# urw7rs/diffusion-models-made-easy

Measured on AMD Instinct MI355X. Metric: denoising steps/sec + training images/sec, DDPM UNet CIFAR10 32×32 @1/2/4/8 GPU, higher is better.
Workload: dtype bf16; 1 GPU; DDPM T=1000 sampling, CIFAR10 32x32, default UNet (32,416,643 params, random init), batch 128 per GPU, t.shape=(1,); global_batch=128, parallelism=dp1 (independent chains per GPU, no data-path collective)

## Files before the change

### diffusion-models-made-easy_amd/csrc/conv1x1_as.hip

```cpp
#include <stdio.h>

#include "conv_common.h"

namespace dmme {

typedef unsigned u32x4_as __attribute__((ext_vector_type(4)));
typedef __attribute__((address_space(3))) u32x4_as lds_u32x4_as;
typedef __attribute__((address_space(3))) f32x4 lds_f32x4_as;

__host__ __device__ constexpr int as_stage_bytes(bool res) { return res ? 128 * 256 : 128 * 128; }
__host__ __device__ constexpr int as_ring(bool res) { return res ? 2 : 3; }

__host__ __device__ inline int as_fold_bytes(int Cout) { return (Cout * 4 + 1023) & ~1023; }

__device__ __forceinline__ void as_swap32(float& x, float& y) {
#if defined(__HIP_DEVICE_COMPILE__)
    asm volatile("s_nop 1\n\tv_permlane32_swap_b32 %0, %1" : "+v"(x), "+v"(y));
#endif
}
__device__ __forceinline__ void as_mfma_drain() {
#if defined(__HIP_DEVICE_COMPILE__)
    asm volatile("s_nop 15\n\ts_nop 7" ::: "memory");
#endif
}

__device__ __forceinline__ float as_sum_rows(float s) {
    s += __builtin_bit_cast(float, __builtin_amdgcn_update_dpp(0, __builtin_bit_cast(int, s), 0x128, 0xf, 0xf, true));
    s += __builtin_bit_cast(float, __builtin_amdgcn_ds_swizzle(__builtin_bit_cast(int, s), 0x401F));
    float lo = s, hi = s;
    as_swap32(lo, hi);
    return lo + hi;
}
__device__ __forceinline__ float as_sum_slots(float s, int nv) {
    if (nv >= 2) s += __builtin_bit_cast(float, __builtin_amdgcn_update_dpp(0, __builtin_bit_cast(int, s), 0xB1, 0xf, 0xf, true));
    if (nv == 4) s += __builtin_bit_cast(float, __builtin_amdgcn_update_dpp(0, __builtin_bit_cast(int, s), 0x4E, 0xf, 0xf, true));
    return s;
}

__device__ __forceinline__ void as_barrier() {
#if defined(__HIP_DEVICE_COMPILE__)
    asm volatile("s_barrier" ::: "memory");
#endif
}

template <int K, typename T>
__device__ __forceinline__ void as_prologue_tile(char* ldsA, const float* par, int tid, bool silu, bool dm) {
    typedef typename Vec8<T>::type bf16x8;
    typedef __attribute__((address_space(3))) u32x4_as lv4;
    typedef __attribute__((address_space(3))) f32x4 lf4;
    const lds_c* P3 = (const lds_c*)par;
#pragma unroll 1
    for (int it = tid; it < 128 * (K / 8); it += 512) {
        const int piece = it & 7, row = (it >> 3) & 127, c = it >> 10;
        const int ch = c * 64 + ((piece ^ ((row >> 1) & 7)) << 3);
        lv4* p = (lv4*)(lds_c*)(ldsA + it * 16);
        bf16x8 x = __builtin_bit_cast(bf16x8, *p);
        float v[8];
#pragma unroll
        for (int e = 0; e < 8; e += 4) {
            const f32x4 sc = *(const lf4*)(P3 + (ch + e) * 4), sh = *(const lf4*)(P3 + (K + ch + e) * 4);
#pragma unroll
            for (int j = 0; j < 4; ++j) v[e + j] = fmaf((float)x[e + j], sc[j], sh[j]);
        }
        if (silu) {
#pragma unroll
            for (int e = 0; e < 8; ++e) v[e] = silu_fast(v[e]);
        }
        if (dm) {
#pragma unroll
            for (int e = 0; e < 8; e += 4) {
                const f32x4 m = *(const lf4*)(P3 + (2 * K + ch + e) * 4);
#pragma unroll
                for (int j = 0; j < 4; ++j) v[e + j] *= m[j];
            }
        }
#pragma unroll
        for (int e = 0; e < 8; ++e) x[e] = (T)v[e];
        *p = __builtin_bit_cast(u32x4_as, x);
    }
}

template <int KCH, bool RES, typename T = bf16>
__global__ void __launch_bounds__(512) conv1x1_as_kernel(ConvArgs a, int HW, int NU) {
    typedef typename Vec8<T>::type bf16x8;
    constexpr int K = 64 * KCH, NKS = 4 * KCH;
    constexpr int RING = as_ring(RES), STAGE = as_stage_bytes(RES);
    constexpr int U_BYTES = 64 * KCH * ROW_DATA;
    constexpr int DPU = 2 * KCH;
    extern __shared__ __attribute__((aligned(16))) char lds[];
    const int tid = threadIdx.x, lane = tid & 63, wave = __builtin_amdgcn_readfirstlane(tid >> 6);
#define AS_STAMP(K) do { if (a.stamps && blockIdx.x < 2 && (threadIdx.x & 255) == 0) a.stamps[blockIdx.x * 32 + (threadIdx.x >> 8) * 16 + (K)] = (long long)wall_clock64(); } while (0)
    AS_STAMP(0);
    const int p0 = blockIdx.x * 128;
    float* foldL = reinterpret_cast<float*>(lds + RING * U_BYTES);
    char* stageL = lds + RING * U_BYTES + as_fold_bytes(a.Cout);
    char* ldsA = RES ? stageL : lds + U_BYTES;
    const bool has_pro = a.scale || a.dmask || a.pro_silu;
    float* parL = reinterpret_cast<float*>(RES ? lds + U_BYTES : stageL);

    if (wave >= 4) {
        const int t = tid - 256, sw = wave - 4;
        for (int c = t; c < a.Cout; c += 256) foldL[c] = (a.bias ? a.bias[c] : 0.f) + (a.tproj ? a.tproj[c] : 0.f);
        if (has_pro && t < K) {
            const int n = p0 / HW, so = n * K + t;
            float sc = 1.f, sh = 0.f;
            if (a.has_gni) {
                gn_in_scale_shift(a, n, t, K, p0 == n * HW, sc, sh);
            } else if (a.scale) {
                sc = a.scale[so];
                sh = a.shift[so];
            }
            parL[t] = sc;
            parL[K + t] = sh;
            parL[2 * K + t] = a.dmask ? a.dmask[so] : 1.f;
        }
        wait_lgkm_all();
        as_barrier();
        if (has_pro) {
            as_prologue_tile<K, T>(ldsA, parL, tid, a.pro_silu != 0, a.dmask != nullptr);
            wait_lgkm_all();
            as_barrier();
        }
        as_barrier();
        const int slot8 = lane & 7;
        const T* res = (const T*)a.res1;
        T* dst = (T*)a.dst;
        const int cgs = a.gn_cg, nv = cgs >> 3;
        int64_t goff[4];
        int soff[4];
#pragma unroll
        for (int q = 0; q < 4; ++q) {
            const int px = 32 * sw + 8 * q + (lane >> 3);
            goff[q] = (int64_t)(p0 + px) * a.Cout + slot8 * 8;
            soff[q] = RES ? px * 256 + ((slot8 ^ (px & 7)) << 5) : px * 128 + ((slot8 ^ (px & 7)) << 4);
        }
#pragma unroll 1
        for (int u = 0; u < NU; ++u) {
            uint4 rv[4];
            if constexpr (RES) {
#pragma unroll
                for (int q = 0; q < 4; ++q) rv[q] = *reinterpret_cast<const uint4*>(res + goff[q] + u * 64);
            }
            as_barrier();
            if (u < 3) AS_STAMP(4 + 3 * u);
            const char* st = stageL + (u & 1) * STAGE;
            float xs[4][8];
            float s1 = 0.f, s1b = 0.f;
#pragma unroll
            for (int q = 0; q < 4; ++q) {
                uint4 raw;
                if constexpr (RES) {
                    const f32x4 v0 = *reinterpret_cast<const f32x4*>(st + soff[q]), v1 = *reinterpret_cast<const f32x4*>(st + soff[q] + 16);
                    const bf16x8 y = __builtin_bit_cast(bf16x8, rv[q]);
                    bf16x8 o;
#pragma unroll
                    for (int e = 0; e < 4; ++e) {
                        o[e] = (T)(v0[e] + (float)y[e]);
                        o[4 + e] = (T)(v1[e] + (float)y[4 + e]);
                    }
                    raw = __builtin_bit_cast(uint4, o);
                } else {
                    raw = *reinterpret_cast<const uint4*>(st + soff[q]);
                }
                *reinterpret_cast<uint4*>(dst + goff[q] + u * 64) = raw;
                if (a.gn_part) {
                    const bf16x8 o = __builtin_bit_cast(bf16x8, raw);
#pragma unroll
                    for (int e = 0; e < 8; ++e) {
                        xs[q][e] = (float)o[e];
                        if (e < 4) s1 += xs[q][e];
                        else s1b += xs[q][e];
                    }
                }
            }
            if (a.gn_part && cgs == 4) {
                const float meanA = as_sum_rows(s1) * (1.f / 128.f), meanB = as_sum_rows(s1b) * (1.f / 128.f);
                float qa = 0.f, qb = 0.f;
#pragma unroll
                for (int q = 0; q < 4; ++q)
#pragma unroll
                    for (int e = 0; e < 4; ++e) {
                        const float da = xs[q][e] - meanA, db = xs[q][4 + e] - meanB;
                        qa = fmaf(da, da, qa);
                        qb = fmaf(db, db, qb);
                    }
                const float m2A = as_sum_rows(qa), m2B = as_sum_rows(qb);
                if (lane < 8) {
                    const int pw = p0 + 32 * sw, n = pw / HW, tile_s = (pw - n * HW) >> 5;
                    const int G = a.Cout / 4, g_first = (u * 64 + lane * 8) / 4;
                    float* o = a.gn_part + (((int64_t)n * a.gn_tiles + tile_s) * G + g_first) * 2;
                    *reinterpret_cast<f32x4*>(o) = f32x4{meanA, m2A, meanB, m2B};
                }
            } else if (a.gn_part) {
                s1 += s1b;
                const float mean = as_sum_slots(as_sum_rows(s1), nv) * (1.f / (float)(32 * cgs));
                float q2 = 0.f;
#pragma unroll
                for (int q = 0; q < 4; ++q)
#pragma unroll
                    for (int e = 0; e < 8; ++e) {
                        const float d = xs[q][e] - mean;
                        q2 = fmaf(d, d, q2);
                    }
                const float m2 = as_sum_slots(as_sum_rows(q2), nv);
                if (lane < 8 && (lane & (nv - 1)) == 0) {
                    const int pw = p0 + 32 * sw, n = pw / HW, tile_s = (pw - n * HW) >> 5;
                    const int G = a.Cout / cgs, c_first = u * 64 + lane * 8;
                    float* o = a.gn_part + (((int64_t)n * a.gn_tiles + tile_s) * G + c_first / cgs) * 2;
                    *reinterpret_cast<f32x2*>(o) = f32x2{mean, m2};
                }
            }
            if (u < 3) AS_STAMP(5 + 3 * u);
        }
        AS_STAMP(13);
        return;
    }

    const int r = lane & 31, h = lane >> 5;
    const int pm = wave >> 1, cn = wave & 1;
    const unsigned ring_base = (unsigned)__builtin_amdgcn_readfirstlane((int)(unsigned)(size_t)(lds_c*)lds);
    const unsigned a_base = (unsigned)__builtin_amdgcn_readfirstlane((int)(unsigned)(size_t)(lds_c*)ldsA);
    unsigned boff[DPU];
#pragma unroll
    for (int i = 0; i < DPU; ++i) {
        const int I = wave + 4 * i, c = I >> 3, row = 8 * (I & 7) + (lane >> 3);
        boff[i] = (unsigned)(row * K + c * 64 + ((lane & 7) ^ ((row >> 1) & 7)) * 8) * 2u;
    }
    auto dma_unit = [&](int u, int slot) __attribute__((always_inline)) {
        const char* sb = (const char*)a.w + (int64_t)u * 64 * K * 2;
#pragma unroll
        for (int i = 0; i < DPU; ++i) glds16_hidden_s(sb, boff[i], ring_base + (unsigned)(slot * U_BYTES + (wave + 4 * i) * 1024));
    };
#pragma unroll
    for (int i = 0; i < 4 * KCH; ++i) {
        const int I = wave + 4 * i, c = I >> 4, row = 8 * (I & 15) + (lane >> 3);
        const int c0 = c * 64;
        const bool second = c0 >= a.C1;
        const T* sbase = second ? (const T*)a.src2 : (const T*)a.src1;
        const int Cs = second ? a.C2 : a.C1, cb = second ? c0 - a.C1 : c0;
        glds16_hidden(sbase + (int64_t)(p0 + row) * Cs + cb + ((lane & 7) ^ ((row >> 1) & 7)) * 8, a_base + (unsigned)(I * 1024));
    }
    dma_unit(0, 0);
    AS_STAMP(1);
    wait_vm_keep<0>();
    as_barrier();
    AS_STAMP(2);

    if (has_pro) {
        as_prologue_tile<K, T>(ldsA, parL, tid, a.pro_silu != 0, a.dmask != nullptr);
        wait_lgkm_all();
        as_barrier();
    }
    uint4 af[2][NKS];
    {
        const lds_c* A3 = (const lds_c*)ldsA;
#pragma unroll
        for (int mi = 0; mi < 2; ++mi) {
            const int row = pm * 64 + mi * 32 + r;
            const int t = row * ROW_DATA + ((h ^ ((row >> 1) & 7)) << 4);
#pragma unroll
            for (int ks = 0; ks < NKS; ++ks)
                af[mi][ks] = __builtin_bit_cast(uint4, *reinterpret_cast<const lds_u32x4_as*>(A3 + (ks >> 2) * (128 * ROW_DATA) + (t ^ ((ks & 3) << 5))));
        }
    }
    AS_STAMP(3);
    wait_vm_keep<0>();
    as_barrier();
    if (NU > 1) dma_unit(1, 1);
    if (RING > 2 && NU > 2) dma_unit(2, 2);

    const int tB = (cn * 32 + r) * ROW_DATA + ((h ^ (((cn * 32 + r) >> 1) & 7)) << 4);
    uint4 bfr[2][4];
#define AS_READ(SET, SLOT, KG)                                                                                                     \
    do {                                                                                                                           \
        const lds_c* rb_ = (const lds_c*)(size_t)(ring_base + (unsigned)((SLOT) * U_BYTES + (KG) * (64 * ROW_DATA)));              \
        _Pragma("unroll") for (int kk = 0; kk < 4; ++kk)                                                                           \
            bfr[SET][kk] = __builtin_bit_cast(uint4, *reinterpret_cast<const lds_u32x4_as*>(rb_ + (tB ^ (kk << 5))));               \
    } while (0)
    const lds_c* F3 = (const lds_c*)foldL;
    f32x16 fold;
#define AS_FOLD(U)                                                                                                                 \
    _Pragma("unroll") for (int g = 0; g < 4; ++g) {                                                                                \
        const f32x4 t_ = *reinterpret_cast<const lds_f32x4_as*>(F3 + ((U) * 64 + cn * 32 + 8 * g + 4 * h) * 4);                    \
        fold[4 * g] = t_[0];                                                                                                       \
        fold[4 * g + 1] = t_[1];                                                                                                   \
        fold[4 * g + 2] = t_[2];                                                                                                   \
        fold[4 * g + 3] = t_[3];                                                                                                   \
    }
    AS_READ(0, 0, 0);
    AS_FOLD(0);
    int slot = 0;
    const int px = pm * 64 + lane;
    char* stw = stageL + px * (RES ? 256 : 128);
    int stoff[4];
#pragma unroll
    for (int g = 0; g < 4; ++g) stoff[g] = ((cn * 4 + g) ^ (px & 7)) << (RES ? 5 : 4);
#pragma unroll 1
    for (int u = 0; u < NU; ++u) {
        const int nslot = slot == RING - 1 ? 0 : slot + 1;
        f32x16 acc[2];
#pragma unroll
        for (int kg = 0; kg < KCH; ++kg) {
            if (kg + 1 < KCH) {
                if (kg & 1)
                    AS_READ(0, slot, kg + 1);
                else
                    AS_READ(1, slot, kg + 1);
            }
#pragma unroll
            for (int kk = 0; kk < 4; ++kk)
#pragma unroll
                for (int mi = 0; mi < 2; ++mi)
                {
                    if (kg == 0 && kk == 0) acc[mi] = fold;
                    mma16<T>(__builtin_bit_cast(uint4, bfr[kg & 1][kk]), __builtin_bit_cast(uint4, af[mi][4 * kg + kk]), acc[mi]);
                }
        }
        if (u < 3) AS_STAMP(4 + 3 * u);
        char* st = stw + (u & 1) * STAGE;
        as_mfma_drain();
#pragma unroll
        for (int g = 0; g < 4; ++g) {
            float v[8];
#pragma unroll
            for (int i = 0; i < 4; ++i) {
                float x = acc[0][4 * g + i], y = acc[1][4 * g + i];
                as_swap32(x, y);
                v[i] = x;
                v[4 + i] = y;
            }
            if constexpr (RES) {
                *reinterpret_cast<f32x4*>(st + stoff[g]) = f32x4{v[0], v[1], v[2], v[3]};
                *reinterpret_cast<f32x4*>(st + stoff[g] + 16) = f32x4{v[4], v[5], v[6], v[7]};
            } else {
                bf16x8 o;
#pragma unroll
                for (int e = 0; e < 8; ++e) o[e] = (T)v[e];
                *reinterpret_cast<bf16x8*>(st + stoff[g]) = o;
            }
        }
        if (RING > 2 && u + RING - 1 < NU)
            wait_vm_keep<(RING - 2) * DPU>();
        else
            wait_vm_keep<0>();
        as_barrier();
        if (u < 3) AS_STAMP(5 + 3 * u);
        if (u + 1 < NU) {
            AS_READ(0, nslot, 0);
            AS_FOLD(u + 1);
            if (u + RING < NU) dma_unit(u + RING, slot);
        }
        slot = nslot;
    }
    AS_STAMP(13);
#undef AS_READ
#undef AS_FOLD
#undef AS_STAMP
}

static bool as_stats_cg_ok(int cg) { return cg == 4 || cg == 8 || cg == 16 || cg == 32; }

static bool as_shape_ok(int dtype, const ConvArgs& a) {
    const bool off = getenv("DMME_NO_CONV1X1_AS") != nullptr;
    constexpr int min_units = 2;
    if (off || !is16(dtype) || a.x3 || a.mix) return false;
    if (a.taps != 1 || a.stride != 1 || a.up || a.in_nchw || a.out_nchw || a.out_silu || a.res2 || a.n_gno) return false;
    if (a.tproj && a.nt != 1) return false;
    const int K = a.C1 + a.C2;
    if ((K != 128 && K != 256) || a.C1 % 64 || a.Cout % 64 || a.Cout / 64 < min_units || a.Cout > 2048) return false;
    if (a.res1 && a.R1 != a.Cout) return false;
    constexpr int min_wgs = 128, max_wgs = 1 << 30;
    const int64_t M = (int64_t)a.N * a.Hout * a.Wout;
    if (M % 128 || M * a.Cout >= (1ll << 30)) return false;
    if (M / 128 < min_wgs || M / 128 > max_wgs) return false;
    if ((a.scale || a.dmask || a.pro_silu) && (a.Hout * a.Wout) % 128) return false;
    return true;
}

bool conv1x1_as_route(int dtype, const ConvArgs& a, ConvRoute& r) {
    if (!as_shape_ok(dtype, a)) return false;
    if (a.gn_part && (!as_stats_cg_ok(a.gn_cg) || (a.Hout * a.Wout) % 32)) return false;
    r = make_route(CONV1X1_AS, 128, 64, 8);
    r.stat_bn = r.stat_px = 32;
    r.stat_tiles = (a.Hout * a.Wout) % 32 ? 0 : a.Hout * a.Wout / 32;
    return true;
}

template <int KCH, bool RES, typename T>
static int launch_as_inst_t(const ConvArgs& a, size_t lds, hipStream_t s) {
    static bool attr_done = false;
    if (!attr_done) {
        DMME_CHECK_HIP(hipFuncSetAttribute(reinterpret_cast<const void*>(conv1x1_as_kernel<KCH, RES, T>), hipFuncAttributeMaxDynamicSharedMemorySize, 160 * 1024));
        attr_done = true;
    }
    const int64_t M = (int64_t)a.N * a.Hout * a.Wout;
    hipLaunchKernelGGL((conv1x1_as_kernel<KCH, RES, T>), dim3((unsigned)(M / 128)), dim3(512), lds, s, a, a.Hout * a.Wout, a.Cout / 64);
    DMME_CHECK_LAUNCH();
    return DMME_OK;
}
template <int KCH, bool RES>
static int launch_as_inst(const ConvArgs& a, size_t lds, hipStream_t s) {
    return a.f16 ? launch_as_inst_t<KCH, RES, f16>(a, lds, s) : launch_as_inst_t<KCH, RES, bf16>(a, lds, s);
}

int launch_conv1x1_as(const ConvArgs& a, hipStream_t s) {
    const int KCH = (a.C1 + a.C2) / 64;
    const bool res = a.res1 != nullptr;
    const size_t lds = (size_t)as_ring(res) * 64 * KCH * ROW_DATA + as_fold_bytes(a.Cout) + 2 * as_stage_bytes(res);
    DMME_REQUIRE(lds <= 160 * 1024, DMME_ERR_UNSUPPORTED, "conv1x1_as: LDS");
    if (KCH == 4) return res ? launch_as_inst<4, true>(a, lds, s) : launch_as_inst<4, false>(a, lds, s);
    return res ? launch_as_inst<2, true>(a, lds, s) : launch_as_inst<2, false>(a, lds, s);
}

}
```

### diffusion-models-made-easy_amd/csrc/kernels_generic.hip

```cpp
#include <stdlib.h>

#include <algorithm>

#include "common.h"

namespace dmme {

template <typename T>
__global__ void __launch_bounds__(256) conv_generic_kernel(ConvArgs a) {
    const int64_t total = (int64_t)a.N * a.Hout * a.Wout * a.Cout;
    const int Cin = a.C1 + a.C2;
    const int Hv = a.up ? 2 * a.Hin : a.Hin, Wv = a.up ? 2 * a.Win : a.Win;
    const int k = a.taps == 9 ? 3 : 1, pad = a.taps == 9 ? 1 : 0;
    for (int64_t idx = blockIdx.x * (int64_t)blockDim.x + threadIdx.x; idx < total;
         idx += (int64_t)gridDim.x * blockDim.x) {
        const int co = (int)(idx % a.Cout);
        int64_t p = idx / a.Cout;
        const int ow = (int)(p % a.Wout);
        p /= a.Wout;
        const int oh = (int)(p % a.Hout);
        const int n = (int)(p / a.Hout);
        const T* w = (const T*)a.w + (int64_t)co * a.taps * Cin;
        const float* sc = a.scale ? a.scale + (int64_t)n * Cin : nullptr;
        const float* sh = a.scale ? a.shift + (int64_t)n * Cin : nullptr;
        const float* dm = a.dmask ? a.dmask + (int64_t)n * Cin : nullptr;
        float acc = 0.f;
        for (int kh = 0; kh < k; ++kh) {
            const int iy = oh * a.stride - pad + kh;
            if (iy < 0 || iy >= Hv) continue;
            if (a.up == 2 && (iy & 1)) continue;
            const int sy = a.up ? (iy >> 1) : iy;
            for (int kw = 0; kw < k; ++kw) {
                const int ix = ow * a.stride - pad + kw;
                if (ix < 0 || ix >= Wv) continue;
                if (a.up == 2 && (ix & 1)) continue;
                const int sx = a.up ? (ix >> 1) : ix;
                const T* wt = w + (kh * k + kw) * Cin;
                const int64_t pix = ((int64_t)n * a.Hin + sy) * a.Win + sx;
                for (int ci = 0; ci < Cin; ++ci) {
                    float v;
                    if (a.in_nchw)
                        v = ((const float*)a.src1)[(((int64_t)n * a.C1 + ci) * a.Hin + sy) * a.Win + sx];
                    else if (ci < a.C1)
                        v = to_f(((const T*)a.src1)[pix * a.C1 + ci]);
                    else
                        v = to_f(((const T*)a.src2)[pix * a.C2 + (ci - a.C1)]);
                    if (sc) v = fmaf(v, sc[ci], sh[ci]);
                    if (a.pro_silu) v = silu_f(v);
                    if (dm) v *= dm[ci];
                    if (!a.in_nchw) v = to_f(from_f<T>(v));
                    acc = fmaf(v, to_f(wt[ci]), acc);
                }
            }
        }
        if (a.bias) acc += a.bias[co];
        if (a.tproj) acc += a.tproj[(int64_t)(a.nt == 1 ? 0 : n) * a.tproj_ld + co];
        const int64_t opix = ((int64_t)n * a.Hout + oh) * a.Wout + ow;
        if (a.res1) {
            if (co < a.R1)
                acc += to_f(((const T*)a.res1)[opix * a.R1 + co]);
            else
                acc += to_f(((const T*)a.res2)[opix * (a.Cout - a.R1) + (co - a.R1)]);
        }
        if (a.out_silu) acc = silu_f(acc);
        if (a.out_nchw)
            ((float*)a.dst)[(((int64_t)n * a.Cout + co) * a.Hout + oh) * a.Wout + ow] = acc;
        else
            ((T*)a.dst)[opix * a.Cout + co] = from_f<T>(acc);
    }
}

template <typename T>
__global__ void __launch_bounds__(256) conv_in_kernel(ConvArgs a, int px_per_block) {
    extern __shared__ __attribute__((aligned(16))) float wl[];
    const int Cin = a.C1, K = 9 * Cin, Cout = a.Cout;
    for (int e = threadIdx.x; e < K * Cout; e += blockDim.x) {
        const int co = e / K, k = e % K;
        wl[k * Cout + co] = to_f(((const T*)a.w)[e]);
    }
    __syncthreads();
    const int tpp = Cout / 8;
    const int ppb = 256 / tpp;
    const int cg = (threadIdx.x % tpp) * 8;
    const int64_t npix = (int64_t)a.N * a.Hout * a.Wout;
    const int64_t p0 = (int64_t)blockIdx.x * px_per_block;
    for (int pp = threadIdx.x / tpp; pp < px_per_block; pp += ppb) {
        const int64_t p = p0 + pp;
        if (p >= npix) break;
        const int ox = (int)(p % a.Wout), oy = (int)((p / a.Wout) % a.Hout), n = (int)(p / ((int64_t)a.Wout * a.Hout));
        float acc[8];
#pragma unroll
        for (int j = 0; j < 8; ++j) acc[j] = a.bias ? a.bias[cg + j] : 0.f;
        for (int kh = 0; kh < 3; ++kh) {
            const int iy = oy - 1 + kh;
            if (iy < 0 || iy >= a.Hin) continue;
            for (int kw = 0; kw < 3; ++kw) {
                const int ix = ox - 1 + kw;
                if (ix < 0 || ix >= a.Win) continue;
                for (int ci = 0; ci < Cin; ++ci) {
                    const float v = a.in_nchw ? ((const float*)a.src1)[(((int64_t)n * Cin + ci) * a.Hin + iy) * a.Win + ix]
                                              : to_f(((const T*)a.src1)[(((int64_t)n * a.Hin + iy) * a.Win + ix) * Cin + ci]);
                    const float* wr = wl + ((kh * 3 + kw) * Cin + ci) * Cout + cg;
                    const float4 w0 = *reinterpret_cast<const float4*>(wr), w1 = *reinterpret_cast<const float4*>(wr + 4);
                    acc[0] = fmaf(v, w0.x, acc[0]); acc[1] = fmaf(v, w0.y, acc[1]);
                    acc[2] = fmaf(v, w0.z, acc[2]); acc[3] = fmaf(v, w0.w, acc[3]);
                    acc[4] = fmaf(v, w1.x, acc[4]); acc[5] = fmaf(v, w1.y, acc[5]);
                    acc[6] = fmaf(v, w1.z, acc[6]); acc[7] = fmaf(v, w1.w, acc[7]);
                }
            }
        }
        T* o = (T*)a.dst + p * Cout + cg;
#pragma unroll
        for (int j = 0; j < 8; ++j) o[j] = from_f<T>(acc[j]);
    }
}

typedef float f32x16_g __attribute__((ext_vector_type(16)));
typedef float f32x4_g __attribute__((ext_vector_type(4)));
template <typename T, int CT>
__global__ void __launch_bounds__(256) conv_in_mfma_kernel(ConvArgs a, int nblocks) {
    const int lane = threadIdx.x & 63, r = lane & 31, h = lane >> 5;
    const int Cin = a.C1, K = 9 * Cin;
    float wreg[CT][14];
#pragma unroll
    for (int ct = 0; ct < CT; ++ct)
#pragma unroll
        for (int j = 0; j < 14; ++j) {
            const int k = 2 * j + h;
            wreg[ct][j] = k < K ? to_f(((const T*)a.w)[(int64_t)(ct * 32 + r) * K + k]) : 0.f;
        }
    const int HW = a.Hout * a.Wout;
    int t_off[14], t_dy[14], t_dx[14];
#pragma unroll
    for (int j = 0; j < 14; ++j) {
        const int k = 2 * j + h, tap = k / Cin, ci = k - tap * Cin;
        t_dy[j] = k < K ? tap / 3 - 1 : 1 << 20;
        t_dx[j] = tap % 3 - 1;
        t_off[j] = (ci * a.Hin + (tap / 3 - 1)) * a.Win + tap % 3 - 1;
    }
    __shared__ __attribute__((aligned(16))) float biasL[128];
    if (threadIdx.x < 32 * CT) biasL[threadIdx.x] = a.bias ? a.bias[threadIdx.x] : 0.f;
    __syncthreads();
    for (int blk = blockIdx.x * 4 + (threadIdx.x >> 6); blk < nblocks; blk += gridDim.x * 4) {
        const int p = blk * 32 + r;
        const int n = p / HW, rem = p - n * HW, oy = rem / a.Wout, ox = rem - oy * a.Wout;
        const float* xb = (const float*)a.src1 + ((int64_t)n * Cin * a.Hin + oy) * a.Win + ox;
        float xv[14];
#pragma unroll
        for (int j = 0; j < 14; ++j) {
            const bool in = (unsigned)(oy + t_dy[j]) < (unsigned)a.Hin && (unsigned)(ox + t_dx[j]) < (unsigned)a.Win;
            xv[j] = in ? xb[t_off[j]] : 0.f;
        }
        constexpr int PITCH = CT * 32 + 4;
        __shared__ __attribute__((aligned(16))) unsigned short stage_in[4][32 * PITCH];
        unsigned short* st = stage_in[threadIdx.x >> 6];
#pragma unroll
        for (int ct = 0; ct < CT; ++ct) {
            f32x16_g acc;
#pragma unroll
            for (int g4 = 0; g4 < 4; ++g4) {
                const f32x4_g b4 = *reinterpret_cast<const f32x4_g*>(biasL + ct * 32 + 8 * g4 + 4 * h);
                acc[4 * g4] = b4[0];
                acc[4 * g4 + 1] = b4[1];
                acc[4 * g4 + 2] = b4[2];
                acc[4 * g4 + 3] = b4[3];
            }
#pragma unroll
            for (int j = 0; j < 14; ++j) acc = __builtin_amdgcn_mfma_f32_32x32x2f32(wreg[ct][j], xv[j], acc, 0, 0, 0);
            if constexpr (sizeof(T) == 2) {
#pragma unroll
                for (int gq = 0; gq < 4; ++gq) {
                    typedef T bf16x4_g __attribute__((ext_vector_type(4)));
                    bf16x4_g v;
#pragma unroll
                    for (int e = 0; e < 4; ++e) v[e] = (T)acc[4 * gq + e];
                    *reinterpret_cast<bf16x4_g*>(st + r * PITCH + ct * 32 + 8 * gq + 4 * h) = v;
                    if (a.gn_part) {
                        float s = 0.f, ss = 0.f;
#pragma unroll
                        for (int e = 0; e < 4; ++e) {
                            const float x = (float)v[e];
                            s += x;
                            ss = fmaf(x, x, ss);
                        }
                        s = half_sum(s);
                        ss = half_sum(ss);
                        if (r == 0) {
                            const float mean = s * (1.f / 128.f);
                            float* po = a.gn_part + (((int64_t)n * a.gn_tiles + (rem >> 5)) * (a.Cout / 4) + ct * 8 + 2 * gq + h) * 2;
                            po[0] = mean;
                            po[1] = ss - s * mean;
                        }
                    }
                }
            } else {
                T* o = (T*)a.dst + (int64_t)p * a.Cout + ct * 32 + 4 * h;
#pragma unroll
                for (int gq = 0; gq < 4; ++gq)
                    *reinterpret_cast<float4*>(o + 8 * gq) = make_float4(acc[4 * gq], acc[4 * gq + 1], acc[4 * gq + 2], acc[4 * gq + 3]);
                if (a.gn_part) {
#pragma unroll
                    for (int gq = 0; gq < 4; ++gq) {
                        float s = 0.f, ss = 0.f;
#pragma unroll
                        for (int e = 0; e < 4; ++e) {
                            const float x = acc[4 * gq + e];
                            s += x;
                            ss = fmaf(x, x, ss);
                        }
                        s = half_sum(s);
                        ss = half_sum(ss);
                        if (r == 0) {
                            const float mean = s * (1.f / 128.f);
                            float* po = a.gn_part + (((int64_t)n * a.gn_tiles + (rem >> 5)) * (a.Cout / 4) + ct * 8 + 2 * gq + h) * 2;
                            po[0] = mean;
                            po[1] = ss - s * mean;
                        }
                    }
                }
            }
        }
        if constexpr (sizeof(T) == 2) {
            __builtin_amdgcn_wave_barrier();
            constexpr int VPR = CT * 4;
#pragma unroll
            for (int q = 0; q < 32 * VPR / 64; ++q) {
                const int it = lane + 64 * q, px = it / VPR, sg = it % VPR;
                const uint2 lo = *reinterpret_cast<const uint2*>(st + px * PITCH + sg * 8), hi = *reinterpret_cast<const uint2*>(st + px * PITCH + sg * 8 + 4);
                *reinterpret_cast<uint4*>((T*)a.dst + (int64_t)(blk * 32 + px) * a.Cout + sg * 8) = make_uint4(lo.x, lo.y, hi.x, hi.y);
            }
            __builtin_amdgcn_wave_barrier();
        }
    }
}

static bool conv_in_mfma_supported(const ConvArgs& a) {
    return a.in_nchw && !a.out_nchw && a.taps == 9 && a.stride == 1 && !a.up && a.C2 == 0 && a.C1 <= 3 && !a.scale && !a.pro_silu && !a.dmask &&
           !a.tproj && !a.res1 && !a.out_silu && (a.Cout == 128 || a.Cout == 64 || a.Cout == 32) &&
           (!a.gn_part || (a.gn_cg == 4 && (a.Hout * a.Wout) % 32 == 0)) &&
           ((int64_t)a.N * a.Hout * a.Wout) % 32 == 0 && (int64_t)a.N * a.Hout * a.Wout * a.Cout < (1ll << 31) && !debug_route("no_conv_in_mfma");
}

void conv_generic_route(const ConvArgs& a, ConvRoute& r) {
    r = make_route(CONV_GENERIC);
    if (!conv_in_mfma_supported(a) || (a.Hout * a.Wout) % 32) return;
    r.vec = r.stat_bn = 4;
    r.stat_px = 32;
    r.stat_tiles = a.Hout * a.Wout / 32;
}

static bool conv_in_supported(const ConvArgs& a) {
    return !a.out_nchw && a.taps == 9 && a.stride == 1 && !a.up && a.C2 == 0 && a.C1 <= 8 && !a.scale &&
           !a.pro_silu && !a.dmask && !a.tproj && !a.res1 && !a.out_silu && a.Cout % 8 == 0 && a.Cout <= 2048 &&
           256 % (a.Cout / 8) == 0 && (size_t)9 * a.C1 * a.Cout * 4 <= 48 * 1024;
}

const char* conv_generic_kernel_name(const ConvArgs& a) {
    return conv_in_mfma_supported(a) ? "conv_in_mfma_kernel" : conv_in_supported(a) ? "conv_in_kernel" : "conv_generic_kernel";
}

int launch_conv_generic(int dtype, const ConvArgs& a, hipStream_t s) {
    if (conv_in_mfma_supported(a)) {
        const int nblocks = (int)((int64_t)a.N * a.Hout * a.Wout / 32);
        unsigned grid = (unsigned)((nblocks + 3) / 4);
        if (grid > 512u) grid = 512u;
#define DMME_CIN(TT, CT) hipLaunchKernelGGL((conv_in_mfma_kernel<TT, CT>), dim3(grid), dim3(256), 0, s, a, nblocks)
        if (dtype == DMME_BF16) {
            if (a.Cout == 128) DMME_CIN(bf16, 4); else if (a.Cout == 64) DMME_CIN(bf16, 2); else DMME_CIN(bf16, 1);
        } else if (dtype == DMME_F16) {
            if (a.Cout == 128) DMME_CIN(f16, 4); else if (a.Cout == 64) DMME_CIN(f16, 2); else DMME_CIN(f16, 1);
        } else {
            if (a.Cout == 128) DMME_CIN(float, 4); else if (a.Cout == 64) DMME_CIN(float, 2); else DMME_CIN(float, 1);
        }
#undef DMME_CIN
        DMME_CHECK_LAUNCH();
        return DMME_OK;
    }
    if (conv_in_supported(a) && !a.gn_part) {
        const int64_t npix = (int64_t)a.N * a.Hout * a.Wout;
        const int ppb = 256 / (a.Cout / 8) * 8;
        const unsigned blocks = (unsigned)((npix + ppb - 1) / ppb);
        const size_t lds = (size_t)9 * a.C1 * a.Cout * 4;
        if (dtype == DMME_BF16)
            hipLaunchKernelGGL(conv_in_kernel<bf16>, dim3(blocks), dim3(256), lds, s, a, ppb);
        else if (dtype == DMME_F16)
            hipLaunchKernelGGL(conv_in_kernel<f16>, dim3(blocks), dim3(256), lds, s, a, ppb);
        else
            hipLaunchKernelGGL(conv_in_kernel<float>, dim3(blocks), dim3(256), lds, s, a, ppb);
        DMME_CHECK_LAUNCH();
        return DMME_OK;
    }
    const int64_t total = (int64_t)a.N * a.Hout * a.Wout * a.Cout;
    if (total == 0) return DMME_OK;
    int64_t blocks = (total + 255) / 256;
    if (blocks > 65536) blocks = 65536;
    if (dtype == DMME_BF16)
        hipLaunchKernelGGL(conv_generic_kernel<bf16>, dim3((unsigned)blocks), dim3(256), 0, s, a);
    else if (dtype == DMME_F16)
        hipLaunchKernelGGL(conv_generic_kernel<f16>, dim3((unsigned)blocks), dim3(256), 0, s, a);
    else
        hipLaunchKernelGGL(conv_generic_kernel<float>, dim3((unsigned)blocks), dim3(256), 0, s, a);
    DMME_CHECK_LAUNCH();
    return DMME_OK;
}

template <typename T>
__global__ void __launch_bounds__(256) gn_generic_kernel(const T* __restrict__ s1, const T* __restrict__ s2, int HW,
                                                         int C1, int C2, int groups, const float* gamma,
                                                         const float* beta, float eps, float* scale, float* shift,
                                                         float* mean_rstd) {
    __shared__ float red[16];
    const int n = blockIdx.y, g = blockIdx.x;
    const int C = C1 + C2, cg = C / groups;
    const int64_t cnt = (int64_t)cg * HW;
    auto at = [&](int64_t e) -> float {
        const int c = g * cg + (int)(e % cg);
        const int64_t p = (int64_t)n * HW + e / cg;
        return c < C1 ? to_f(s1[p * C1 + c]) : to_f(s2[p * C2 + (c - C1)]);
    };
    float s = 0.f;
    for (int64_t e = threadIdx.x; e < cnt; e += blockDim.x) s += at(e);
    const float mean = block_sum(s, red) / (float)cnt;
    float q = 0.f;
    for (int64_t e = threadIdx.x; e < cnt; e += blockDim.x) {
        const float d = at(e) - mean;
        q = fmaf(d, d, q);
    }
    const float var = block_sum(q, red) / (float)cnt;
    const float rstd = 1.0f / sqrtf(var + eps);
    if (mean_rstd && threadIdx.x == 0) {
        mean_rstd[((int64_t)n * groups + g) * 2] = mean;
        mean_rstd[((int64_t)n * groups + g) * 2 + 1] = rstd;
    }
    for (int j = threadIdx.x; j < cg; j += blockDim.x) {
        const int c = g * cg + j;
        const float a = rstd * gamma[c];
        scale[(int64_t)n * C + c] = a;
        shift[(int64_t)n * C + c] = beta[c] - mean * a;
    }
}

int launch_gn_generic(int dtype, const void* src1, const void* src2, int N, int HW, int C1, int C2, int groups,
                      const float* gamma, const float* beta, float eps, float* scale, float* shift, float* mean_rstd,
                      hipStream_t s) {
    dim3 grid(groups, N);
    if (dtype == DMME_BF16)
        hipLaunchKernelGGL(gn_generic_kernel<bf16>, grid, dim3(256), 0, s, (const bf16*)src1, (const bf16*)src2, HW,
                           C1, C2, groups, gamma, beta, eps, scale, shift, mean_rstd);
    else if (dtype == DMME_F16)
        hipLaunchKernelGGL(gn_generic_kernel<f16>, grid, dim3(256), 0, s, (const f16*)src1, (const f16*)src2, HW,
                           C1, C2, groups, gamma, beta, eps, scale, shift, mean_rstd);
    else
        hipLaunchKernelGGL(gn_generic_kernel<float>, grid, dim3(256), 0, s, (const float*)src1, (const float*)src2,
                           HW, C1, C2, groups, gamma, beta, eps, scale, shift, mean_rstd);
    DMME_CHECK_LAUNCH();
    return DMME_OK;
}

template <typename T>
__global__ void __launch_bounds__(256) attn_generic_kernel(const T* __restrict__ qkv, int S, int C, int heads, int N, T* __restrict__ out) {
    extern __shared__ __attribute__((aligned(16))) float sm[];
    const int d = C / heads;
    float* qs = sm;
    float* ps = sm + d;
    float* red = ps + S;
    const int bh = blockIdx.y, n = bh / heads, hd = bh % heads, i = blockIdx.x;
    const T* base = qkv + (int64_t)n * S * 3 * C + (int64_t)hd * 3 * d;
    const float kscale = powf((float)C, -0.5f);
    for (int c = threadIdx.x; c < d; c += blockDim.x) qs[c] = to_f(base[(int64_t)i * 3 * C + c]);
    __syncthreads();
    float lmax = -INFINITY;
    for (int j = threadIdx.x; j < S; j += blockDim.x) {
        const T* kr = base + (int64_t)j * 3 * C + d;
        float acc = 0.f;
        for (int c = 0; c < d; ++c) acc = fmaf(qs[c], to_f(from_f<T>(to_f(kr[c]) * kscale)), acc);
        ps[j] = acc;
        lmax = fmaxf(lmax, acc);
    }
    const float m = block_max(lmax, red);
    float lsum = 0.f;
    for (int j = threadIdx.x; j < S; j += blockDim.x) {
        const float e = expf(ps[j] - m);
        ps[j] = e;
        lsum += e;
    }
    const float tot = block_sum(lsum, red);
    __syncthreads();
    const float inv = 1.0f / tot;
    const int on = bh % N, oh = bh / N;
    for (int c = threadIdx.x; c < d; c += blockDim.x) {
        float acc = 0.f;
        for (int j = 0; j < S; ++j) acc = fmaf(to_f(from_f<T>(ps[j] * inv)), to_f(base[(int64_t)j * 3 * C + 2 * d + c]), acc);
        out[((int64_t)on * S + i) * C + oh * d + c] = from_f<T>(acc);
    }
}

template <typename T>
__global__ void __launch_bounds__(256) attn_s16_kernel(const T* __restrict__ qkv, int C, int heads, int N, T* __restrict__ out) {
    extern __shared__ __attribute__((aligned(16))) float sm[];
    constexpr int S = 16;
    const int d = C / heads, dp = d + 4;
    float* qs = sm;
    float* ks = qs + S * dp;
    float* vs = ks + S * dp;
    float* ps = vs + S * dp;
    const int bh = blockIdx.x, n = bh / heads, hd = bh % heads, tid = threadIdx.x;
    const T* base = qkv + (int64_t)n * S * 3 * C + (int64_t)hd * 3 * d;
    const float kscale = powf((float)C, -0.5f);
    for (int e = tid; e < S * d; e += 256) {
        const int row = e / d, c = e - row * d;
        const T* p = base + (int64_t)row * 3 * C + c;
        qs[row * dp + c] = to_f(p[0]);
        ks[row * dp + c] = to_f(from_f<T>(to_f(p[d]) * kscale));
        vs[row * dp + c] = to_f(p[2 * d]);
    }
    __syncthreads();
    const int i = tid >> 4, j = tid & 15;
    float acc = 0.f;
    for (int c = 0; c < d; c += 4) {
        const f32x4_g a = *reinterpret_cast<const f32x4_g*>(qs + i * dp + c), b = *reinterpret_cast<const f32x4_g*>(ks + j * dp + c);
        acc = fmaf(a[0], b[0], acc);
        acc = fmaf(a[1], b[1], acc);
        acc = fmaf(a[2], b[2], acc);
        acc = fmaf(a[3], b[3], acc);
    }
    float m = acc;
    m = fmaxf(m, DMME_DPP_F(m, 0xB1));
    m = fmaxf(m, DMME_DPP_F(m, 0x4E));
    m = fmaxf(m, DMME_DPP_F(m, 0x141));
    m = fmaxf(m, DMME_DPP_F(m, 0x140));
    const float e = expf(acc - m);
    const float tot = row16_sum(e);
    ps[i * 17 + j] = to_f(from_f<T>(e * (1.0f / tot)));
    __syncthreads();
    const int on = bh % N, oh = bh / N;
    for (int c = j; c < d; c += 16) {
        float o = 0.f;
#pragma unroll
        for (int jj = 0; jj < S; ++jj) o = fmaf(ps[i * 17 + jj], vs[jj * dp + c], o);
        out[((int64_t)on * S + i) * C + oh * d + c] = from_f<T>(o);
    }
}

int launch_attn_heads(int dtype, const void* qkv, int N, int S, int C, int heads, void* out, hipStream_t s) {
    DMME_REQUIRE(heads >= 1 && C % heads == 0, DMME_ERR_INVALID, "attention: width %d not divisible by %d heads", C, heads);
    if (S == 16 && (C / heads) % 4 == 0 && C / heads <= 1024 && !debug_route("no_attn_s16")) {
        const size_t lds16 = (size_t)(3 * 16 * (C / heads + 4) + 16 * 17) * sizeof(float);
        if (lds16 <= 64 * 1024) {
            if (dtype == DMME_BF16)
                hipLaunchKernelGGL(attn_s16_kernel<bf16>, dim3((unsigned)(N * heads)), dim3(256), lds16, s, (const bf16*)qkv, C, heads, N, (bf16*)out);
            else if (dtype == DMME_F16)
                hipLaunchKernelGGL(attn_s16_kernel<f16>, dim3((unsigned)(N * heads)), dim3(256), lds16, s, (const f16*)qkv, C, heads, N, (f16*)out);
            else
                hipLaunchKernelGGL(attn_s16_kernel<float>, dim3((unsigned)(N * heads)), dim3(256), lds16, s, (const float*)qkv, C, heads, N, (float*)out);
            DMME_CHECK_LAUNCH();
            return DMME_OK;
        }
    }
    const size_t lds = (size_t)(C / heads + S + 16) * sizeof(float);
    DMME_REQUIRE(lds <= 64 * 1024, DMME_ERR_UNSUPPORTED, "attention generic: d+S too large (%d+%d)", C / heads, S);
    dim3 grid(S, N * heads);
    if (dtype == DMME_BF16)
        hipLaunchKernelGGL(attn_generic_kernel<bf16>, grid, dim3(256), lds, s, (const bf16*)qkv, S, C, heads, N, (bf16*)out);
    else if (dtype == DMME_F16)
        hipLaunchKernelGGL(attn_generic_kernel<f16>, grid, dim3(256), lds, s, (const f16*)qkv, S, C, heads, N, (f16*)out);
    else
        hipLaunchKernelGGL(attn_generic_kernel<float>, grid, dim3(256), lds, s, (const float*)qkv, S, C, heads, N, (float*)out);
    DMME_CHECK_LAUNCH();
    return DMME_OK;
}
int launch_attn_generic(int dtype, const void* qkv, int N, int S, int C, void* out, hipStream_t s) {
    return launch_attn_heads(dtype, qkv, N, S, C, 1, out, s);
}

__global__ void gn_modulate_kernel(float* __restrict__ scale, float* __restrict__ shift, const float* __restrict__ t_shift,
                                   const float* __restrict__ t_scale, int ld, int nt, int N, int C) {
    const int i = blockIdx.x * blockDim.x + threadIdx.x;
    if (i >= N * C) return;
    const int n = i / C, c = i % C, r = nt == 1 ? 0 : n;
    const float m = 1.0f + t_scale[(int64_t)r * ld + c];
    scale[i] = scale[i] * m;
    shift[i] = fmaf(shift[i], m, t_shift[(int64_t)r * ld + c]);
}
int launch_gn_modulate(float* scale, float* shift, const float* t_shift, const float* t_scale, int ld, int nt, int N, int C, hipStream_t s) {
    hipLaunchKernelGGL(gn_modulate_kernel, dim3((N * C + 255) / 256), dim3(256), 0, s, scale, shift, t_shift, t_scale, ld, nt, N, C);
    DMME_CHECK_LAUNCH();
    return DMME_OK;
}

__global__ void time_sinusoid_kernel(const int64_t* t, int nt, const float* freqs, int half, float* out, unsigned* mark, unsigned mark_val) {
    const int i = blockIdx.x * blockDim.x + threadIdx.x;
    if (i == 0 && mark) *mark = mark_val;
    if (i >= nt * half) return;
    const int r = i / half, k = i % half;
    const float arg = (float)t[r] * freqs[k];
// ... 615 lines not shown
```

Measured before the change: 469.6 denoising steps/s (one step = UNet forward + DDPM update on a batch of 128), summed over GPUs.

## Deepen LDS prefetch in conv1x1 and software-pipeline input loads in generic conv

```diff
diff --git a/diffusion-models-made-easy_amd/csrc/conv1x1_as.hip b/diffusion-models-made-easy_amd/csrc/conv1x1_as.hip
--- a/diffusion-models-made-easy_amd/csrc/conv1x1_as.hip
+++ b/diffusion-models-made-easy_amd/csrc/conv1x1_as.hip
@@ -16,11 +16,6 @@
 __device__ __forceinline__ void as_swap32(float& x, float& y) {
 #if defined(__HIP_DEVICE_COMPILE__)
     asm volatile("s_nop 1\n\tv_permlane32_swap_b32 %0, %1" : "+v"(x), "+v"(y));
-#endif
-}
-__device__ __forceinline__ void as_mfma_drain() {
-#if defined(__HIP_DEVICE_COMPILE__)
-    asm volatile("s_nop 15\n\ts_nop 7" ::: "memory");
 #endif
 }
 
@@ -270,7 +265,7 @@
     if (RING > 2 && NU > 2) dma_unit(2, 2);
 
     const int tB = (cn * 32 + r) * ROW_DATA + ((h ^ (((cn * 32 + r) >> 1) & 7)) << 4);
-    uint4 bfr[2][4];
+    uint4 bfr[3][4];
 #define AS_READ(SET, SLOT, KG)                                                                                                     \
     do {                                                                                                                           \
         const lds_c* rb_ = (const lds_c*)(size_t)(ring_base + (unsigned)((SLOT) * U_BYTES + (KG) * (64 * ROW_DATA)));              \
@@ -288,57 +283,46 @@
         fold[4 * g + 3] = t_[3];                                                                                                   \
     }
     AS_READ(0, 0, 0);
+    AS_READ(1, 0, 1);
     AS_FOLD(0);
     int slot = 0;
-    const int px = pm * 64 + lane;
-    char* stw = stageL + px * (RES ? 256 : 128);
+    char* stw = stageL + (pm * 64 + r) * (RES ? 256 : 128);
     int stoff[4];
 #pragma unroll
-    for (int g = 0; g < 4; ++g) stoff[g] = ((cn * 4 + g) ^ (px & 7)) << (RES ? 5 : 4);
+    for (int g = 0; g < 4; ++g) stoff[g] = (((cn * 4 + g) ^ (r & 7)) << (RES ? 5 : 4)) + h * (RES ? 16 : 8);
 #pragma unroll 1
     for (int u = 0; u < NU; ++u) {
         const int nslot = slot == RING - 1 ? 0 : slot + 1;
         f32x16 acc[2];
 #pragma unroll
         for (int kg = 0; kg < KCH; ++kg) {
-            if (kg + 1 < KCH) {
-                if (kg & 1)
-                    AS_READ(0, slot, kg + 1);
-                else
-                    AS_READ(1, slot, kg + 1);
-            }
+            if (kg + 2 < KCH) AS_READ((kg + 2) % 3, slot, kg + 2);
 #pragma unroll
             for (int kk = 0; kk < 4; ++kk)
 #pragma unroll
                 for (int mi = 0; mi < 2; ++mi)
                 {
                     if (kg == 0 && kk == 0) acc[mi] = fold;
-                    mma16<T>(__builtin_bit_cast(uint4, bfr[kg & 1][kk]), __builtin_bit_cast(uint4, af[mi][4 * kg + kk]), acc[mi]);
+                    mma16<T>(__builtin_bit_cast(uint4, bfr[kg % 3][kk]), __builtin_bit_cast(uint4, af[mi][4 * kg + kk]), acc[mi]);
                 }
         }
         if (u < 3) AS_STAMP(4 + 3 * u);
         char* st = stw + (u & 1) * STAGE;
-        as_mfma_drain();
-#pragma unroll
-        for (int g = 0; g < 4; ++g) {
-            float v[8];
-#pragma unroll
-            for (int i = 0; i < 4; ++i) {
-                float x = acc[0][4 * g + i], y = acc[1][4 * g + i];
-                as_swap32(x, y);
-                v[i] = x;
-                v[4 + i] = y;
-            }
-            if constexpr (RES) {
-                *reinterpret_cast<f32x4*>(st + stoff[g]) = f32x4{v[0], v[1], v[2], v[3]};
-                *reinterpret_cast<f32x4*>(st + stoff[g] + 16) = f32x4{v[4], v[5], v[6], v[7]};
-            } else {
-                bf16x8 o;
-#pragma unroll
-                for (int e = 0; e < 8; ++e) o[e] = (T)v[e];
-                *reinterpret_cast<bf16x8*>(st + stoff[g]) = o;
-            }
-        }
+#pragma unroll
+        for (int mi = 0; mi < 2; ++mi)
+#pragma unroll
+            for (int g = 0; g < 4; ++g) {
+                char* q = st + mi * 32 * (RES ? 256 : 128) + stoff[g];
+                if constexpr (RES) {
+                    *reinterpret_cast<f32x4*>(q) = f32x4{acc[mi][4 * g], acc[mi][4 * g + 1], acc[mi][4 * g + 2], acc[mi][4 * g + 3]};
+                } else {
+                    typedef T bf16x4_as __attribute__((ext_vector_type(4)));
+                    bf16x4_as o;
+#pragma unroll
+                    for (int e = 0; e < 4; ++e) o[e] = (T)acc[mi][4 * g + e];
+                    *reinterpret_cast<bf16x4_as*>(q) = o;
+                }
+            }
         if (RING > 2 && u + RING - 1 < NU)
             wait_vm_keep<(RING - 2) * DPU>();
         else
@@ -347,6 +331,7 @@
         if (u < 3) AS_STAMP(5 + 3 * u);
         if (u + 1 < NU) {
             AS_READ(0, nslot, 0);
+            AS_READ(1, nslot, 1);
             AS_FOLD(u + 1);
             if (u + RING < NU) dma_unit(u + RING, slot);
         }
diff --git a/diffusion-models-made-easy_amd/csrc/kernels_generic.hip b/diffusion-models-made-easy_amd/csrc/kernels_generic.hip
--- a/diffusion-models-made-easy_amd/csrc/kernels_generic.hip
+++ b/diffusion-models-made-easy_amd/csrc/kernels_generic.hip
@@ -127,7 +127,8 @@
 #pragma unroll
         for (int j = 0; j < 14; ++j) {
             const int k = 2 * j + h;
-            wreg[ct][j] = k < K ? to_f(((const T*)a.w)[(int64_t)(ct * 32 + r) * K + k]) : 0.f;
+            const float wv = to_f(((const T*)a.w)[(int64_t)(ct * 32 + r) * K + (k < K ? k : 0)]);
+            wreg[ct][j] = k < K ? wv : 0.f;
         }
     const int HW = a.Hout * a.Wout;
     int t_off[14], t_dy[14], t_dx[14];
@@ -141,16 +142,29 @@
     __shared__ __attribute__((aligned(16))) float biasL[128];
     if (threadIdx.x < 32 * CT) biasL[threadIdx.x] = a.bias ? a.bias[threadIdx.x] : 0.f;
     __syncthreads();
-    for (int blk = blockIdx.x * 4 + (threadIdx.x >> 6); blk < nblocks; blk += gridDim.x * 4) {
-        const int p = blk * 32 + r;
+    auto load_x = [&](int b, float (&x)[14], unsigned& inside) __attribute__((always_inline)) {
+        const int p = b * 32 + r;
         const int n = p / HW, rem = p - n * HW, oy = rem / a.Wout, ox = rem - oy * a.Wout;
         const float* xb = (const float*)a.src1 + ((int64_t)n * Cin * a.Hin + oy) * a.Win + ox;
-        float xv[14];
+        inside = 0u;
 #pragma unroll
         for (int j = 0; j < 14; ++j) {
             const bool in = (unsigned)(oy + t_dy[j]) < (unsigned)a.Hin && (unsigned)(ox + t_dx[j]) < (unsigned)a.Win;
-            xv[j] = in ? xb[t_off[j]] : 0.f;
-        }
+            x[j] = xb[in ? t_off[j] : 0];
+            inside |= in ? 1u << j : 0u;
+        }
+    };
+    const int blk0 = blockIdx.x * 4 + (threadIdx.x >> 6), bstep = gridDim.x * 4;
+    float xn[14];
+    unsigned in_n = 0u;
+    if (blk0 < nblocks) load_x(blk0, xn, in_n);
+    for (int blk = blk0; blk < nblocks; blk += bstep) {
+        const int p = blk * 32 + r;
+        const int n = p / HW, rem = p - n * HW;
+        float xv[14];
+#pragma unroll
+        for (int j = 0; j < 14; ++j) xv[j] = (in_n >> j) & 1u ? xn[j] : 0.f;
+        if (blk + bstep < nblocks) load_x(blk + bstep, xn, in_n);
         constexpr int PITCH = CT * 32 + 4;
         __shared__ __attribute__((aligned(16))) unsigned short stage_in[4][32 * PITCH];
         unsigned short* st = stage_in[threadIdx.x >> 6];
@@ -168,6 +182,7 @@
 #pragma unroll
             for (int j = 0; j < 14; ++j) acc = __builtin_amdgcn_mfma_f32_32x32x2f32(wreg[ct][j], xv[j], acc, 0, 0, 0);
             if constexpr (sizeof(T) == 2) {
+                float s[4], ss[4];
 #pragma unroll
                 for (int gq = 0; gq < 4; ++gq) {
                     typedef T bf16x4_g __attribute__((ext_vector_type(4)));
@@ -175,22 +190,28 @@
 #pragma unroll
                     for (int e = 0; e < 4; ++e) v[e] = (T)acc[4 * gq + e];
                     *reinterpret_cast<bf16x4_g*>(st + r * PITCH + ct * 32 + 8 * gq + 4 * h) = v;
-                    if (a.gn_part) {
-                        float s = 0.f, ss = 0.f;
-#pragma unroll
-                        for (int e = 0; e < 4; ++e) {
-                            const float x = (float)v[e];
-                            s += x;
-                            ss = fmaf(x, x, ss);
+                    s[gq] = ss[gq] = 0.f;
+#pragma unroll
+                    for (int e = 0; e < 4; ++e) {
+                        const float x = (float)v[e];
+                        s[gq] += x;
+                        ss[gq] = fmaf(x, x, ss[gq]);
+                    }
+                }
+                if (a.gn_part) {
+                    float mean = 0.f, m2 = 0.f;
+#pragma unroll
+                    for (int gq = 0; gq < 4; ++gq) {
+                        const float sg = half_sum(s[gq]), ssg = half_sum(ss[gq]);
+                        const float mg = sg * (1.f / 128.f), qg = ssg - sg * mg;
+                        if (r == gq) {
+                            mean = mg;
+                            m2 = qg;
                         }
-                        s = half_sum(s);
-                        ss = half_sum(ss);
-                        if (r == 0) {
-                            const float mean = s * (1.f / 128.f);
-                            float* po = a.gn_part + (((int64_t)n * a.gn_tiles + (rem >> 5)) * (a.Cout / 4) + ct * 8 + 2 * gq + h) * 2;
-                            po[0] = mean;
-                            po[1] = ss - s * mean;
-                        }
+                    }
+                    if (r < 4) {
+                        float* po = a.gn_part + (((int64_t)n * a.gn_tiles + (rem >> 5)) * (a.Cout / 4) + ct * 8 + 2 * r + h) * 2;
+                        *reinterpret_cast<float2*>(po) = make_float2(mean, m2);
                     }
                 }
             } else {
```

Measured after the change: 469.5 denoising steps/s (one step = UNet forward + DDPM update on a batch of 128), summed over GPUs. About the same (-0.0%).
